# jimonld2000/AudioDenoiser

Hardware: AMD Instinct MI355X
Metric: spectrogram frames/sec (forward), 513x256 fp32 (higher is better)
Workload: dtype f32; 1 GPU; BASELINE configs[1]: batch=64 synthetic 513x256 fp32 spectrograms on one MI355X, full U-Net forward + per-clip perceptual loss; batch_per_gpu=64, global_batch=64, freq_bins=513, frames=256, parallelism=clips sharded over 1 rank(s), weights replicated, no data-path collective, lib_digest=ac1cc53c7748

## Files before the change

audiodenoiser_amd/csrc/adn_internal.h:

```cpp
#pragma once
#include <hip/hip_runtime.h>
#include <atomic>
#include <cstddef>
#include <cstdint>
#include <type_traits>

namespace adn {

template <typename T> constexpr int ACT_BLOCK = 32 / (int)sizeof(T);
template <typename T>
__host__ __device__ __forceinline__ long act_off(int C, long HW, long pix, int c)
{
    constexpr int B = ACT_BLOCK<T>;
    (void)C;
    return ((long)(c / B) * HW + pix) * B + (c % B);
}

#ifdef __HIPCC__
typedef float f32x2 __attribute__((ext_vector_type(2)));
typedef float f32x4 __attribute__((ext_vector_type(4)));
typedef float f32x16 __attribute__((ext_vector_type(16)));
typedef _Float16 f16x2 __attribute__((ext_vector_type(2)));
typedef _Float16 f16x4 __attribute__((ext_vector_type(4)));
typedef _Float16 f16x8 __attribute__((ext_vector_type(8)));
// ... 206 lines not shown
    return hipSuccess;
}
inline int device_cus()
{
    static std::atomic<int> cus{0};
    int c = cus.load(std::memory_order_relaxed);
    if (c == 0) {
        int dev = 0;
        if (hipGetDevice(&dev) != hipSuccess || hipDeviceGetAttribute(&c, hipDeviceAttributeMultiprocessorCount, dev) != hipSuccess || c < 8)
            return 0;
        c &= ~7;
        cus.store(c, std::memory_order_relaxed);
    }
    return c;
}

hipError_t launch_conv_mfma(ConvKind kind, const ConvArgs &a, bool f16, hipStream_t st);
hipError_t launch_conv_reduce(ConvKind kind, const ConvArgs &a, bool f16, hipStream_t st);
hipError_t launch_convt_reduce(const float *partial, const float *bias, float *out, int ksplit, int N, int Ho, int Wo, int Cout,
                               hipStream_t st);
constexpr int WINO_BN = 32;
hipError_t launch_wino_conv(ConvKind kind, const ConvArgs &a, hipStream_t st);
long wino_tiles(ConvArgs &a);
bool wino4_applicable(ConvKind kind, const ConvArgs &a, bool force);
long wino4_workgroups(const ConvArgs &a);
hipError_t launch_wino4_conv(ConvKind kind, const ConvArgs &a, hipStream_t st);

struct Wino3sGeom {
    int tilesY, tilesX;
    long rows;
    size_t v_bytes, m_bytes;
    long gemm_grid;
};
bool wino3s_applicable(ConvKind kind, const ConvArgs &a);
Wino3sGeom wino3s_geom(const ConvArgs &a);
hipError_t launch_wino3s_conv(ConvKind kind, const ConvArgs &a, float *V, float *M, hipStream_t st);
hipError_t launch_wino_gemm(const float *V, const void *U, float *M, long rows, int Cin, int Cout, hipStream_t st);

bool conv16_applicable(ConvKind kind, const ConvArgs &a);
hipError_t launch_conv16(ConvKind kind, const ConvArgs &a, bool resident, hipStream_t st);

bool convt16_applicable(const ConvArgs &a);
hipError_t launch_convt16(const ConvArgs &a, hipStream_t st);

hipError_t launch_conv_first(const float *x, const float *w9x64, const float *bias, void *out, bool f16,
                             int N, int H, int W, int Cin, hipStream_t st);
hipError_t launch_dot_finish(const float *planes, int nplanes, float bias, float *y, long npix, hipStream_t st);
hipError_t launch_conv_out(const void *in, bool f16, const float *w64, float bias, float *out, long npix, long HW,
                           long out_stride, hipStream_t st);
hipError_t launch_nhwc_to_nchw(const void *in, bool f16, float *out, int N, int H, int W, int C, hipStream_t st);

hipError_t launch_stft_mag(const float *audio, int n_clips, long L, int n_fft, int hop, int center, long n_frames,
                           float *out, int rows, long row_stride, long clip_stride, int quantize, hipStream_t st);
constexpr hipError_t ADN_COLD_IN_CAPTURE = hipErrorStreamCaptureUnsupported;
bool stream_is_capturing(hipStream_t st);
hipError_t stft_tables(int n_fft, const float **out, hipStream_t st);
hipError_t loss_tables(hipStream_t st);
hipError_t launch_gl_polar(const float *mag, const float *rnd, int n_clips, int F, int T, void *spec, hipStream_t st);
hipError_t launch_istft_frames(const void *spec, int n_clips, int T, int n_fft, float *buf, hipStream_t st);
hipError_t launch_istft_ola(const float *buf, int n_clips, int T, int n_fft, int hop, float *audio, hipStream_t st);
hipError_t launch_stft_complex(const float *audio, int n_clips, long L, int n_fft, int hop, int T, void *spec,
                               hipStream_t st);
struct DenoiseGeom {
    int T, K, Wd, S, V;
};
bool denoise_geom(int n_frames, int window, int overlap, DenoiseGeom *g);
hipError_t launch_denoise_windows(const void *spec, int n_clips, int F, const DenoiseGeom &g, float *out, hipStream_t st);
hipError_t launch_denoise_stitch(const float *y, int n_clips, int F, const DenoiseGeom &g, int clamp, float *out,
                                 hipStream_t st);
hipError_t launch_denoise_resynth(const float *y, const void *spec, int n_clips, long L, int n_fft, int hop,
// ... 167 lines not shown
```

audiodenoiser_amd/csrc/conv_kernels.hip:

```cpp
#include "adn_internal.h"

#include <cstdlib>

namespace adn {

namespace {

constexpr int TW = 16;
constexpr int CONVT_KG = 2, CONVT_WPE = 4;

template <typename T> struct Elem;
template <> struct Elem<float> { static constexpr int EPV = 4; };
template <> struct Elem<_Float16> { static constexpr int EPV = 8; };

template <int TH, int BN, int WM, int WN>
__device__ __forceinline__ void conv_epilogue_raw(const ConvArgs &p, f32x16 (&acc)[TH * TW / 32 / WM][BN / 32 / WN], int lane, int wave,
                                                  int ct, int n, int ty, int tx)
{
    constexpr int MB = TH * TW / 32 / WM, NB = BN / 32 / WN;
    const int wm = wave / WN, wn = wave % WN;
    const int hh = lane >> 5, l31 = lane & 31;
    float *ob = static_cast<float *>(p.out) + (size_t)n * p.H * p.W * p.Cout;
#pragma unroll
    for (int j = 0; j < NB; ++j) {
// ... 250 lines not shown
    for (int j = 0; j < NB; ++j) {
        const int col = (wn * NB + j) * 32 + l31;
        const float bv = bias_r[j];
#pragma unroll
        for (int i = 0; i < MB; ++i) {
            const int pix0 = ((HALVES == 1 ? wm * MB : 0) + i) * 32 + 4 * hh;
            float v[16];
#pragma unroll
            for (int r = 0; r < 16; ++r) {
                v[r] = acc[i][j][r] + bv;
                if (EPI != CONVT2X2 && EPI != WINO_GEMM) v[r] = relu_nan(v[r]);
            }
            if constexpr (sizeof(T) == 4) {
#pragma unroll
                for (int r = 0; r < 16; ++r) stage[(pix0 + (r & 3) + 8 * (r >> 2)) * RS + col] = v[r];
            } else {
                const bool odd = l31 & 1;
#pragma unroll
                for (int r = 0; r < 16; r += 2) {
                    const float send = odd ? v[r] : v[r + 1];
                    const float recv = __shfl_xor(send, 1, 64);
                    const float lo = odd ? recv : v[r], hi = odd ? v[r + 1] : recv;
                    const int pix = pix0 + ((r + (odd ? 1 : 0)) & 3) + 8 * (r >> 2);
                    *reinterpret_cast<f16x2 *>(stage + pix * RS + (col & ~1)) = f16x2{(_Float16)lo, (_Float16)hi};
                }
            }
        }
    }
    }
    __syncthreads();

    T *outp = static_cast<T *>(p.out);
    if constexpr (EPI == CONVT2X2) {
        static_assert(BN == 128 && NT % 64 == 0, "transposed-convolution epilogue: 128 columns per workgroup");
        constexpr int BE = ACT_BLOCK<T>, NBLK = 64 / BE;
        const int Ho = 2 * p.H, Wo = 2 * p.W;
        const int ncg = p.Cout >> 6, di = ct / ncg, cg = ct - di * ncg;
        const size_t bstr = (size_t)Ho * Wo * BE;
        T *ob = outp + (size_t)n * Ho * Wo * p.Cout + (size_t)(NBLK * cg) * bstr;
        const int gxl = lane >> 2, dj = (lane >> 1) & 1, half = lane & 1;
        const int gx = tx * TW + gxl;
        constexpr int THH = TH / HALVES;
#pragma unroll
        for (int it = 0; it < NBLK * THH / (NT / 64); ++it) {
            const int run = it * (NT / 64) + wave;
            const int b8 = run / THH, py = run - b8 * THH;
            const int gy = ty * TH + hf * THH + py;
            const piece_t val = *reinterpret_cast<const piece_t *>(stage + (py * TW + gxl) * RS + dj * 64 + b8 * BE + half * EPP);
            if (gy < p.H && gx < p.W)
                *reinterpret_cast<piece_t *>(ob + b8 * bstr + ((size_t)(2 * gy + di) * Wo + 2 * gx + dj) * BE + half * EPP) = val;
        }
        if (HALVES > 1 && hf + 1 < HALVES) __syncthreads();
    } else if constexpr (EPI == WINO_GEMM) {
        static_assert(sizeof(T) == 4 && BN % 8 == 0, "Winograd GEMM: fp32");
        constexpr int HPIX = NPIX / HALVES;
        T *ob = outp + (size_t)n * p.rows * p.Cout + (size_t)ct * (BN / 8) * p.rows * 8;
#pragma unroll
        for (int it = 0; it < HPIX * PPR / NT; ++it) {
            const int id = it * NT + tid;
            const int b8 = id / (2 * HPIX), rem = id - b8 * (2 * HPIX), pix = rem >> 1, half = rem & 1;
            const long row = (long)ty * NPIX + hf * HPIX + pix;
            if (row < p.rows)
                *reinterpret_cast<piece_t *>(ob + ((size_t)b8 * p.rows + row) * 8 + half * 4) =
                    *reinterpret_cast<const piece_t *>(stage + pix * RS + b8 * 8 + half * 4);
        }
        if (HALVES > 1 && hf + 1 < HALVES) __syncthreads();
    } else if constexpr (EPI == CONV3X3_RELU_DOT) {
        static_assert(PPR <= 64 && (PPR & (PPR - 1)) == 0 && NT % PPR == 0, "pieces of a pixel must sit in one wave");
        float wv[EPP];
#pragma unroll
        for (int e = 0; e < EPP; ++e) wv[e] = p.dotw[(tid % PPR) * EPP + e];
#pragma unroll
        for (int it = 0; it < NPIX * PPR / NT; ++it) {
            const int id = it * NT + tid;
            const int pix = id / PPR, part = id - pix * PPR;
            const int gy = ty * TH + (pix >> 4), gx = tx * TW + (pix & 15);
            const piece_t val = *reinterpret_cast<const piece_t *>(stage + pix * RS + part * EPP);
            float s = 0.f;
#pragma unroll
            for (int e = 0; e < EPP; ++e) s += wv[e] * (float)val[e];
#pragma unroll
            for (int o = PPR / 2; o > 0; o >>= 1) s += __shfl_xor(s, o, 64);
            if (part == 0 && gy < p.H && gx < p.W) p.dot_out[((size_t)n * p.H + gy) * p.W + gx] = s + p.dot_bias;
        }
// ... 481 lines not shown
#pragma unroll
        for (int a = 0; a < 2; ++a)
#pragma unroll
            for (int b = 0; b < 2; ++b) {
                const int gy = 2 * by + a, gx = 2 * bx + b;
                if (gy >= H || gx >= W) continue;
                const f32x4 v = finish(gy, gx);
                mx.x = max_nan(mx.x, v.x); mx.y = max_nan(mx.y, v.y); mx.z = max_nan(mx.z, v.z); mx.w = max_nan(mx.w, v.w);
            }
        if (by < H / 2 && bx < W / 2)
            *reinterpret_cast<Tx4 *>(pool + (size_t)n * (H / 2) * (W / 2) * Cout +
                                     act_off<T>(Cout, (long)(H / 2) * (W / 2), (long)by * (W / 2) + bx, c4)) = as_t(mx);
    }
}

template <typename T>
hipError_t launch_conv_mfma_t(ConvKind kind, const ConvArgs &a, hipStream_t st)
{
    if constexpr (sizeof(T) == 2) {
        if (a.ksplit > 1) {
            if (kind != CONV3X3_RELU) return hipErrorInvalidValue;
            return launch_dma_cfg<T, 32, 64, 8, 1, 9, 1, CONV3X3_RELU, 4, 0, 1>(a, st);
        }
        if (kind == CONVT2X2) return launch_dma_cfg<T, 8, 128, 2, 2, 1, CONVT_KG, CONVT2X2, CONVT_WPE>(a, st);
        if (kind == CONV3X3_RELU_DOT) {
            if (a.nct != 1 || !a.dotw || !a.dot_out) return hipErrorInvalidValue;
            return launch_dma_cfg<T, 32, 64, 8, 1, 9, 1, CONV3X3_RELU_DOT, 4>(a, st);
        }
        if (kind == CONV3X3_RELU_POOL) return launch_dma_cfg<T, 32, 64, 8, 1, 9, 1, CONV3X3_RELU_POOL, 4>(a, st);
        return launch_dma_cfg<T, 32, 64, 8, 1, 9, 1, CONV3X3_RELU, 4>(a, st);
    } else {
        if (kind == CONV3X3_RELU_DOT) return hipErrorInvalidValue;
        if (kind == CONVT2X2) {
            if (a.split && a.ksplit > 1) return launch_dma_cfg<T, 8, 128, 2, 2, 1, CONVT_KG, CONVT2X2, 3, 1, 1>(a, st);
            if (a.ksplit > 1) return hipErrorInvalidValue;
            if (a.split) return launch_dma_cfg<T, 8, 128, 2, 2, 1, CONVT_KG, CONVT2X2, 3, 1>(a, st);
            return launch_dma_cfg<T, 8, 128, 2, 2, 1, CONVT_KG, CONVT2X2, CONVT_WPE>(a, st);
        }
        if (a.Cout == 64) {
            if (kind == CONV3X3_RELU_POOL) return launch_cfg<T, 16, 64, 4, 1, 9, 1, CONV3X3_RELU_POOL>(a, st);
            return launch_cfg<T, 16, 64, 4, 1, 9, 1, CONV3X3_RELU>(a, st);
        }
        if (kind == CONV3X3_RELU_POOL) return launch_cfg<T, 8, 128, 2, 2, 9, 1, CONV3X3_RELU_POOL>(a, st);
        return launch_cfg<T, 8, 128, 2, 2, 9, 1, CONV3X3_RELU>(a, st);
    }
}

}

ConvGeom conv_geom(ConvKind kind, int Cout, bool f16)
{
    const int cpg = f16 ? 16 : 8;
    if (kind == CONVT2X2) return ConvGeom{8, 128, CONVT_KG * cpg};
    if (f16) return ConvGeom{32, 64, cpg};
    if (Cout == 64) return ConvGeom{16, 64, cpg};
    return ConvGeom{8, 128, cpg};
}

long conv_mfma_tiles(ConvKind kind, bool f16, ConvArgs &a)
{
    const ConvGeom g = conv_geom(kind, a.Cout, f16);
    a.tilesY = (a.H + g.TH - 1) / g.TH;
    a.tilesX = (a.W + TW - 1) / TW;
    a.nct = (kind == CONVT2X2 ? 4 * a.Cout : a.Cout) / g.BN;
    return conv_workgroups(a);
}

hipError_t launch_conv_mfma(ConvKind kind, const ConvArgs &a, bool f16, hipStream_t st)
{
    return f16 ? launch_conv_mfma_t<_Float16>(kind, a, st) : launch_conv_mfma_t<float>(kind, a, st);
}

hipError_t launch_wino_gemm(const float *V, const void *U, float *M, long rows, int Cin, int Cout, hipStream_t st)
{
    if (!V || !U || !M || rows < 1 || rows >= (1L << 25) || Cin < 16 || (Cin & 15) || Cout < 128 || (Cout & 127)) return hipErrorInvalidValue;
    ConvArgs a{};
    a.N = 36;
    a.W = TW;
    a.H = (int)((rows + TW - 1) / TW);
    a.rows = rows;
    a.s0 = ConvSrc{V, a.H, a.W, Cin, 0, 0};
    a.s1 = ConvSrc{V, 0, 0, 0, 0, 0};
    a.nchunk0 = a.nchunk = Cin / 16;
    a.wpk = U;
    a.out = M;
    a.Cout = Cout;
    a.ksplit = 1;
    a.split = 1;
    a.tilesY = (a.H + 7) / 8;
    a.tilesX = 1;
    a.nct = Cout / 128;
    return launch_dma_cfg<float, 8, 128, 2, 2, 1, CONVT_KG, WINO_GEMM, 3, 1>(a, st);
}

template <typename T>
static hipError_t launch_conv_reduce_t(bool pl, const ConvArgs &a, unsigned blocks, hipStream_t st)
{
    if (pl)
        hipLaunchKernelGGL((conv_reduce_kernel<T, true>), dim3(blocks), dim3(256), 0, st, a.partial, a.bias, static_cast<T *>(a.out),
                           static_cast<T *>(a.pool), a.ksplit, a.N, a.H, a.W, a.Cout);
    else
        hipLaunchKernelGGL((conv_reduce_kernel<T, false>), dim3(blocks), dim3(256), 0, st, a.partial, a.bias, static_cast<T *>(a.out),
                           static_cast<T *>(nullptr), a.ksplit, a.N, a.H, a.W, a.Cout);
    return hipGetLastError();
}

hipError_t launch_conv_reduce(ConvKind kind, const ConvArgs &a, bool f16, hipStream_t st)
{
    const bool pl = kind == CONV3X3_RELU_POOL;
    if (a.ksplit < 2 || a.ksplit > ADN_MAX_KSPLIT || !a.partial || (a.Cout & (f16 ? 15 : 3)) || (kind != CONV3X3_RELU && !pl) || (pl && !a.pool))
        return hipErrorInvalidValue;
    const long items = pl ? (long)a.N * ((a.H + 1) / 2) * ((a.W + 1) / 2) * (a.Cout / 4) : (long)a.N * a.H * a.W * (a.Cout / 4);
    const long blocks = (items + 255) / 256;
    if (items <= 0 || blocks > 0x7fffffffL) return hipErrorInvalidValue;
    return f16 ? launch_conv_reduce_t<_Float16>(pl, a, (unsigned)blocks, st) : launch_conv_reduce_t<float>(pl, a, (unsigned)blocks, st);
}

hipError_t launch_convt_reduce(const float *partial, const float *bias, float *out, int ksplit, int N, int Ho, int Wo, int Cout,
                               hipStream_t st)
{
    const long n4 = (long)N * Ho * Wo * Cout / 4;
    const long blocks = (n4 + 255) / 256;
    if (ksplit < 2 || ksplit > ADN_MAX_KSPLIT || (Cout & 7) || blocks <= 0 || blocks > 0x7fffffffL) return hipErrorInvalidValue;
    hipLaunchKernelGGL(convt_reduce_kernel, dim3((unsigned)blocks), dim3(256), 0, st, reinterpret_cast<const f32x4 *>(partial), bias,
// ... 69 lines not shown
```

audiodenoiser_amd/csrc/unet.hip:

```cpp
#include "adn_host.h"

#include <algorithm>
#include <cmath>
#include <cstdlib>
#include <cstring>
#include <memory>
#include <vector>

using adn::aligned_to;
using adn::DeviceGuard;
using adn::fail;
using adn::fail_hip;

namespace {

constexpr float BN_EPS = 1e-5f;
constexpr int CH[5] = {64, 128, 256, 512, 1024};

enum LayerKind { CONV3, CONVT };
struct LayerDesc {
    LayerKind kind;
    int level;
    int C0, C1;
    int Cout;
};
constexpr int N_CONV3 = 17, N_CONVT = 4, N_LAYERS = N_CONV3 + N_CONVT;
struct LayerTable {
    LayerDesc v[N_LAYERS];
    int n;
};
constexpr LayerTable make_layers()
{
    LayerTable t{};
    for (int l = 0; l <= 4; ++l) {
        if (l > 0) t.v[t.n++] = LayerDesc{CONV3, l, CH[l - 1], 0, CH[l]};
        t.v[t.n++] = LayerDesc{CONV3, l, CH[l], 0, CH[l]};
    }
    for (int l = 3; l >= 0; --l) {
        t.v[t.n++] = LayerDesc{CONVT, l + 1, CH[l + 1], 0, CH[l]};
        t.v[t.n++] = LayerDesc{CONV3, l, CH[l], CH[l], CH[l]};
        t.v[t.n++] = LayerDesc{CONV3, l, CH[l], 0, CH[l]};
    }
    return t;
}
constexpr LayerTable NET = make_layers();
static_assert(NET.n == N_LAYERS && NET.v[0].Cout == 64 && NET.v[8].C0 == 1024 && NET.v[9].kind == CONVT && NET.v[N_LAYERS - 1].Cout == 64,
              "layer table: 9 layers down to the bottleneck, then 4 x (convT, conv, conv)");
static_assert(6 * (1 + N_CONV3) + 2 * N_CONVT + 2 == ADN_N_WEIGHT_TENSORS, "layer table does not match the weight tensor list");
static_assert(1 + N_LAYERS + 1 == ADN_N_LAUNCHES, "layer table does not match the timing slots");

struct LayerWeights {
    size_t w_off, b_off;
    size_t w4_off;
    size_t w3_off;
    size_t w16_off;
    size_t braw_off;
};

}

struct adn_unet {
    int device = 0;
    float *dev = nullptr;
    size_t dev_floats = 0;
    size_t first_w = 0, first_b = 0;
    LayerWeights lw[N_LAYERS] = {};
    size_t out_w = 0;
    size_t zero_off = 0;
    float out_b = 0.f;
    std::vector<float> out_bias;
    int in_ch = 1, n_classes = 1;
    std::vector<hipEvent_t> events;
    int timing_max = 0, timing_count = 0;
    bool f16 = false;
    bool use_wino = true;
    bool use_wino4 = true, force_wino4 = false;
    bool allow_split = false;
    bool convt_split = true;
    int f16_conv = 1;
    int f16_convt = 1;
    bool f16_fuse_first = true;
    bool batch_invariant = false;
    long auto_grid = 192, auto_grid64 = 512;
    int wino_gemm = 1;
    long gemm_grid = 1536;
};

namespace {

void bn_fold(const float *b, const float *gamma, const float *beta, const float *mean, const float *var, int C,
             std::vector<float> &scale, std::vector<float> &bias)
{
    scale.resize(C);
    bias.resize(C);
    for (int c = 0; c < C; ++c) {
        const float s = gamma[c] / std::sqrt(var[c] + BN_EPS);
        scale[c] = s;
        bias[c] = (b[c] - mean[c]) * s + beta[c];
    }
}

template <typename T>
void pack_conv3x3(const float *w , const std::vector<float> &scale, int Cin, int Cout, T *dst)
{
    constexpr int EPV = 16 / sizeof(T);
    const adn::ConvGeom g = adn::conv_geom(adn::CONV3X3_RELU, Cout, sizeof(T) == 2);
    const int BN = g.BN, KC = g.KC, KG = KC / (2 * EPV);
    const int nct = Cout / BN, nchunk = Cin / KC;
    size_t o = 0;
    for (int ct = 0; ct < nct; ++ct)
        for (int ch = 0; ch < nchunk; ++ch)
            for (int tap = 0; tap < 9; ++tap)
                for (int s = 0; s < KG; ++s)
                    for (int h = 0; h < 2; ++h)
                        for (int n = 0; n < BN; ++n) {
                            const int co = ct * BN + n;
                            for (int kk = 0; kk < EPV; ++kk) {
                                const int ci = ch * KC + 2 * EPV * s + EPV * h + kk;
// ... 105 lines not shown
                            dst[(((((size_t)ct * nchunk + ch) * 16 + cb) * 4 + g) * 16 + c16) * 8 + e] =
                                (_Float16)w[(((size_t)ci * Cout + co) * 2 + di) * 2 + dj];
                        }
            }
}

inline uint16_t bf16_rne(float f)
{
    uint32_t u;
    std::memcpy(&u, &f, 4);
    if ((u & 0x7fffffffu) > 0x7f800000u) return (uint16_t)((u >> 16) | 0x40);
    u += 0x7fffu + ((u >> 16) & 1u);
    return (uint16_t)(u >> 16);
}
inline float bf16_to_float(uint16_t b)
{
    const uint32_t u = (uint32_t)b << 16;
    float f;
    std::memcpy(&f, &u, 4);
    return f;
}
inline void split3_host(float v, uint16_t (&t)[3])
{
    uint16_t hi = bf16_rne(v);
    if ((hi & 0x7fffu) == 0x7f80u && std::isfinite(v)) hi = (uint16_t)((hi & 0x8000u) | 0x7f7fu);
    const float r1 = v - bf16_to_float(hi);
    const uint16_t mid = bf16_rne(r1);
    const float r2 = r1 - bf16_to_float(mid);
    t[0] = hi;
    t[1] = mid;
    t[2] = bf16_rne(r2);
}

void pack_wino4_split(const float *w , const std::vector<float> &scale, int Cin, int Cout, uint16_t *dst)
{
    const int nct = Cout / 128, nchunk = Cin / 16;
    for (int co = 0; co < Cout; ++co)
        for (int ci = 0; ci < Cin; ++ci) {
            float U[36];
            wino4_u(w + ((size_t)co * Cin + ci) * 9, scale[co], U);
            const int ct = co / 128, n = co % 128, ch = ci / 16, hh = (ci % 16) / 8, kk = ci % 8;
            for (int pos = 0; pos < 36; ++pos) {
                uint16_t t[3];
                split3_host(U[pos], t);
                uint16_t *slab = dst + (((size_t)pos * nct + ct) * nchunk + ch) * (3 * 2 * 128 * 8);
                for (int plane = 0; plane < 3; ++plane) slab[((plane * 2 + hh) * 128 + n) * 8 + kk] = t[plane];
            }
        }
}

void pack_convt_split(const float *w , int Cin, int Cout, uint16_t *dst)
{
    const int BN = 128, KC = 16;
    const int ncol = 4 * Cout, nct = ncol / BN, nchunk = Cin / KC;
    size_t o = 0;
    for (int ct = 0; ct < nct; ++ct)
        for (int ch = 0; ch < nchunk; ++ch)
            for (int plane = 0; plane < 3; ++plane)
                for (int h = 0; h < 2; ++h)
                    for (int n = 0; n < BN; ++n) {
                        int ij, co;
                        adn::convt_column(ct * BN + n, Cout, ij, co);
                        for (int kk = 0; kk < 8; ++kk) {
                            const int ci = ch * KC + 8 * h + kk;
                            uint16_t t[3];
                            split3_host(w[((size_t)ci * Cout + co) * 4 + ij], t);
                            dst[o++] = t[plane];
                        }
                    }
}


adn::ConvArgs geom_args(const LayerDesc &d, bool f16, bool wino, int N, int H, int W)
{
    const adn::ConvKind kind = d.kind == CONVT ? adn::CONVT2X2 : adn::CONV3X3_RELU;
    adn::ConvArgs a{};
    a.s0.C = d.C0;
    a.s1.C = d.C1;
    a.N = N;
    a.H = H;
    a.W = W;
    a.Cout = d.Cout;
    a.ksplit = 1;
    const int kc = adn::conv_geom(kind, d.Cout, f16).KC;
    a.nchunk0 = d.C0 / kc;
    a.nchunk = (d.C0 + d.C1) / kc;
// ... 70 lines not shown
    }
    a.wpk = h->dev + L.w_off;
    a.wpk4 = (h->use_wino && h->use_wino4 && L.w4_off) ? h->dev + L.w4_off : (h->f16 && L.w16_off) ? h->dev + L.w16_off : nullptr;
    a.bias = h->dev + L.b_off;
    a.out = out;
    a.pool = pool;
    return a;
}

adn::ConvArgs convt_args(const adn_unet *h, const Plan &p, int i, const void *in, void *out)
{
    const LayerDesc &d = NET.v[i];
    const int H = p.H[d.level], W = p.W[d.level];
    adn::ConvArgs a = geom_args(d, h->f16, false, p.N, H, W);
    a.s0 = adn::ConvSrc{in, H, W, d.C0, 0, 0};
    a.s1 = adn::ConvSrc{in, 0, 0, 0, 0, 0};
    a.wpk = h->dev + h->lw[i].w_off;
    a.bias = h->dev + h->lw[i].b_off;
    a.out = out;
    a.split = h->convt_split ? 1 : 0;
    return a;
}


enum Conv3Kernel {
    DIRECT,
    CONV16,
    WINO2,
    WINO4,
    WINO3S
};
struct WinoScratch {
    const void *U = nullptr;
    float *V = nullptr, *M = nullptr;
    size_t v_bytes = 0, m_bytes = 0;
};
struct Conv3Choice {
    Conv3Kernel kernel;
    int ksplit;
    bool fuse_first;
    bool fuse_out;
};

Conv3Choice choose_conv3(const adn_unet *h, adn::ConvKind kind, const adn::ConvArgs &a, bool first = false, bool tail = false,
                         const WinoScratch &sc = WinoScratch())
{
    Conv3Choice c{DIRECT, 1, false, false};
    if (h->f16) {
        const bool c16 = a.wpk4 && adn::conv16_applicable(kind, a);
        c.fuse_out = tail && a.nct == 1;
        if (first && h->f16_fuse_first && c16) {
            c.kernel = CONV16;
            c.fuse_first = true;
            return c;
        }
        if (a.wpk4 && !h->batch_invariant && !c.fuse_out)
            c.ksplit = adn::conv16_ksplit(adn::conv_workgroups(a), a.nchunk, (size_t)a.N * a.H * a.W * a.Cout);
        if (c.ksplit == 1 && c16) c.kernel = CONV16;
        return c;
    }
    if (!h->use_wino) return c;
    c.kernel = WINO2;
    c.fuse_out = tail && a.nct == 2;
    auto done = [&]() {
        c.fuse_first = first && c.kernel == WINO2 && c.ksplit == 1;
        return c;
// ... 16 lines not shown
        if (fits && (h->wino_gemm == 2 || pinned || (automatic && g3.gemm_grid >= h->gemm_grid))) {
            c.kernel = WINO3S;
            return c;
        }
    }
    if (f4_ok && (!automatic || g4 >= thr)) {
        c.kernel = WINO4;
        return done();
    }
    if (automatic && can_split) c.ksplit = adn::wino_ksplit(g2, a.nchunk);
    if (automatic && can_split && f4_ok) {
        const int ks4 = adn::wino4_ksplit(g4, a.nchunk);
        if (ks4 > 1) {
            const double out_mb = (double)a.N * a.H * a.W * a.Cout * 4.0 * 1e-6;
            auto reduce_us = [&](int ks) { return ks > 1 ? 4.0 + (ks + 1) * out_mb / 8.0 : 0.0; };
            const double t4 = 12.0 + 2.79 * (a.nchunk / ks4) * (double)((g4 * ks4 + 255) / 256) + reduce_us(ks4);
            const double t2 = 8.0 + 2.06 * (a.nchunk / c.ksplit) * (double)((g2 * c.ksplit + 511) / 512) + reduce_us(c.ksplit);
            if (t4 < t2) {
                c.kernel = WINO4;
                c.ksplit = ks4;
            }
        }
    }
    return done();
}

hipError_t launch_conv3_kernels(const adn_unet *h, adn::ConvKind kind, const Conv3Choice &c, adn::ConvArgs a, float *partial, hipStream_t st,
                                const WinoScratch &sc)
{
    if (c.fuse_out) kind = adn::CONV3X3_RELU_DOT;
    switch (c.kernel) {
    case WINO3S:
        a.wpk = sc.U;
        return adn::launch_wino3s_conv(kind, a, sc.V, sc.M, st);
    case CONV16:
        a.wpk = a.wpk4;
        a.nchunk0 = a.s0.C / 32;
        a.nchunk = (a.s0.C + a.s1.C) / 32;
        if (c.fuse_first) a.nchunk0 = a.nchunk = 2;
        return adn::launch_conv16(kind, a, c.fuse_first || (a.s0.C + a.s1.C == 64 && a.Cout == 64), st);
    case DIRECT:
        if (c.ksplit > 1) {
            adn::ConvArgs sl = a;
            sl.ksplit = c.ksplit;
            sl.out = partial;
            sl.pool = nullptr;
            hipError_t e = adn::launch_conv_mfma(adn::CONV3X3_RELU, sl, true, st);
            if (e != hipSuccess) return e;
            a.ksplit = c.ksplit;
            a.partial = partial;
            return adn::launch_conv_reduce(kind, a, true, st);
        }
        return adn::launch_conv_mfma(kind, a, h->f16, st);
    case WINO4:
        a.wpk = a.wpk4;
        [[fallthrough]];
    case WINO2:
        a.ksplit = c.ksplit;
        a.partial = partial;
        return c.kernel == WINO4 ? adn::launch_wino4_conv(kind, a, st) : adn::launch_wino_conv(kind, a, st);
    }
    return hipErrorInvalidValue;
}

inline int hip_status(hipError_t e, const char *what)
{
    return e == hipSuccess ? ADN_OK : fail_hip(e, what);
// ... 19 lines not shown
struct ConvTChoice {
    bool t16;
    int ksplit;
};

ConvTChoice choose_convt(const adn_unet *h, const LayerWeights &L, const adn::ConvArgs &a)
{
    ConvTChoice c{false, 1};
    if (h->f16) {
        c.t16 = L.w16_off && adn::convt16_applicable(a);
        return c;
    }
    if (h->convt_split && !h->batch_invariant)
        c.ksplit = adn::convt_ksplit(adn::conv_workgroups(a), a.nchunk, (size_t)a.N * (2 * a.H) * (2 * a.W) * a.Cout);
    return c;
}

hipError_t launch_convt_kernels(const adn_unet *h, const LayerWeights &L, const ConvTChoice &c, adn::ConvArgs a, float *partial, hipStream_t st)
{
    if (c.t16) {
        a.wpk = h->dev + L.w16_off;
        a.bias = h->dev + L.braw_off;
        return adn::launch_convt16(a, st);
    }
    if (c.ksplit > 1) {
        float *out = static_cast<float *>(a.out);
        a.ksplit = c.ksplit;
        a.out = partial;
        a.bias = h->dev + h->zero_off;
        hipError_t e = adn::launch_conv_mfma(adn::CONVT2X2, a, h->f16, st);
        if (e != hipSuccess) return e;
        return adn::launch_convt_reduce(partial, h->dev + L.braw_off, out, c.ksplit, a.N, 2 * a.H, 2 * a.W, a.Cout, st);
    }
    return adn::launch_conv_mfma(adn::CONVT2X2, a, h->f16, st);
}

int launch_convt(const adn_unet *h, int layer, const ConvTChoice &c, const adn::ConvArgs &a, float *partial, size_t part_bytes, hipStream_t st)
{
    if (int rc = check_part(layer, c.ksplit, (size_t)a.N * (2 * a.H) * (2 * a.W) * a.Cout, part_bytes)) return rc;
    return hip_status(launch_convt_kernels(h, h->lw[layer], c, a, partial, st), "launch_convt");
}


int forward_impl(adn_unet *h, const float *x, float *y, int N, int F, int T, void *workspace, size_t ws_bytes,
                 float *const *taps, hipStream_t st)
{
    if (!h || !x || !y) return fail(ADN_ERR_INVALID, "adn_unet_forward: null handle/x/y");
    Plan p;
    if (!make_plan(N, F, T, h->f16, p)) return fail(ADN_ERR_INVALID, "adn_unet_forward: need N>=1, F,T>=16 and F*T<2^27");
    if (!workspace || ws_bytes < p.total)
        return fail(ADN_ERR_WORKSPACE, "adn_unet_forward: workspace too small (see adn_unet_workspace_bytes)");
    if (!aligned_to(workspace, 16)) return fail(ADN_ERR_INVALID, "adn_unet_forward: workspace must be 16-byte aligned");
    if (!aligned_to(x, 4) || !aligned_to(y, 4)) return fail(ADN_ERR_INVALID, "adn_unet_forward: x and y must be 4-byte aligned");
    DeviceGuard guard(h->device);
    if (guard.err != hipSuccess) return fail_hip(guard.err, "hipSetDevice");

    char *ws = static_cast<char *>(workspace);
    void *tA = ws + p.tA, *tB = ws + p.tB;
    float *part = reinterpret_cast<float *>(ws + p.part);
    const bool f16 = h->f16;
    const bool timed = h->timing_max > 0 && h->timing_count < h->timing_max && !taps;
    hipEvent_t *ev = timed ? h->events.data() + (size_t)h->timing_count * (ADN_N_LAUNCHES + 1) : nullptr;
    int evi = 0;
#define ADN_MARK()                                          \
    do {                                                    \
        if (timed) ADN_HIP(hipEventRecord(ev[evi++], st));  \
    } while (0)
#define ADN_TRY(call)                                       \
    do {                                                    \
        if (int rc_ = (call)) return rc_;                   \
    } while (0)

    auto export_tap = [&](int idx, const void *buf, int layer) -> hipError_t {
        if (!taps || !taps[idx]) return hipSuccess;
        const LayerDesc &d = NET.v[layer];
        return adn::launch_nhwc_to_nchw(buf, f16, taps[idx], N, p.H[d.level], p.W[d.level], d.Cout, st);
    };
    int i = 0;
    auto wino_scratch = [&](int li) {
        WinoScratch sc;
        const LayerDesc &d = NET.v[li];
        if (f16 || !h->lw[li].w3_off) return sc;
        const size_t full = (size_t)N * p.H[0] * p.W[0] * 64 * sizeof(float);
        const size_t front = (size_t)N * p.H[d.level] * p.W[d.level] * std::max(std::max(d.C0, d.C1), d.Cout) * sizeof(float);
        if (front >= full) return sc;
        sc.U = h->dev + h->lw[li].w3_off;
        sc.V = reinterpret_cast<float *>(static_cast<char *>(tA) + front);
        sc.M = reinterpret_cast<float *>(static_cast<char *>(tB) + front);
        sc.v_bytes = sc.m_bytes = full - front;
        return sc;
    };

    const void *cur = tA;
    for (int l = 0; l < 4; ++l) {
        void *skip = ws + p.skip[l], *pool = ws + p.pool[l];
        if (l > 0) {
            const WinoScratch sc = wino_scratch(i);
            const adn::ConvArgs a = conv_args(h, p, i++, ws + p.pool[l - 1], nullptr, 0, 0, tA, nullptr);
            ADN_MARK();
            ADN_TRY(launch_conv3(h, i - 1, adn::CONV3X3_RELU, choose_conv3(h, adn::CONV3X3_RELU, a, false, false, sc), a, part, p.part_bytes, st, sc));
        }
        const WinoScratch sc = wino_scratch(i);
        adn::ConvArgs a = conv_args(h, p, i++, cur, nullptr, 0, 0, skip, pool);
        const Conv3Choice c = choose_conv3(h, adn::CONV3X3_RELU_POOL, a, l == 0 && h->in_ch == 1, false, sc);
        if (l == 0) {
            ADN_MARK();
            if (c.fuse_first) {
                a.s0 = adn::ConvSrc{x, p.H[0], p.W[0], 1, 0, 0};
                a.firstw = h->dev + h->first_w;
                a.firstb = h->dev + h->first_b;
            } else {
                ADN_HIP(adn::launch_conv_first(x, h->dev + h->first_w, h->dev + h->first_b, tA, f16, N, p.H[0], p.W[0], h->in_ch, st));
            }
        }
        ADN_MARK();
        ADN_TRY(launch_conv3(h, i - 1, adn::CONV3X3_RELU_POOL, c, a, part, p.part_bytes, st, sc));
        ADN_HIP(export_tap(l, skip, i - 1));
    }
    {
// ... 60 lines not shown
    if (n_tensors != ADN_N_WEIGHT_TENSORS) return fail(ADN_ERR_INVALID, "adn_unet_create: expected 118 tensors");
    for (int i = 0; i < n_tensors; ++i)
        if (!t[i]) return fail(ADN_ERR_INVALID, "adn_unet_create: null tensor pointer");
    int ndev = 0;
    if (hipGetDeviceCount(&ndev) != hipSuccess || ndev <= 0) return fail(ADN_ERR_NO_DEVICE, "no HIP device visible");
    if (device < 0 || device >= ndev) return fail(ADN_ERR_INVALID, "adn_unet_create: bad device index");
    return ADN_OK;
}

int check_device_arch(int device)
{
    hipDeviceProp_t prop;
    ADN_HIP(hipGetDeviceProperties(&prop, device));
    if (std::strncmp(prop.gcnArchName, "gfx950", 6) != 0)
        return fail(ADN_ERR_NO_DEVICE, std::string("libadn is built for gfx950 only, device is ") + prop.gcnArchName);
    return ADN_OK;
}

void read_switches(adn_unet &h)
{
    if (const char *algo = std::getenv("ADN_CONV_ALGO"))
        h.use_wino = std::strcmp(algo, "direct") != 0;
    if (h.f16) h.use_wino = false;
    if (const char *sk = std::getenv("ADN_WINO_SPLITK")) h.allow_split = std::atoi(sk) != 0;
    if (const char *cs = std::getenv("ADN_CONVT_SPLIT")) h.convt_split = std::atoi(cs) != 0;
    if (const char *bi = std::getenv("ADN_BATCH_INVARIANT")) h.batch_invariant = std::atoi(bi) != 0;
    if (const char *ff = std::getenv("ADN_F16_FIRST")) h.f16_fuse_first = std::atoi(ff) != 0;
    if (const char *fc = std::getenv("ADN_F16_CONV")) h.f16_conv = std::atoi(fc) == 32 ? 0 : 1;
    if (const char *ft = std::getenv("ADN_F16_CONVT")) h.f16_convt = std::strcmp(ft, "dma") == 0 ? 0 : 1;
    if (const char *ag = std::getenv("ADN_AUTO_GRID")) h.auto_grid = std::atol(ag);
    if (const char *ag = std::getenv("ADN_AUTO_GRID64")) h.auto_grid64 = std::atol(ag);
    if (h.f16) h.convt_split = false;
    if (const char *wg = std::getenv("ADN_WINO_GEMM")) h.wino_gemm = std::atoi(wg) == 2 ? 2 : std::atoi(wg) != 0;
    if (const char *wt = std::getenv("ADN_WINO_TILE")) {
        h.use_wino4 = std::atoi(wt) != 2;
        h.force_wino4 = std::atoi(wt) == 4;
    }
}

void pack_weights(adn_unet &h, const float *const *t, std::vector<float> &host)
{
    auto reserve = [&](size_t n) {
        const size_t at = host.size();
        host.resize(at + ((n + 63) & ~size_t(63)), 0.f);
        return at;
    };
    auto halfs = [&](size_t off) { return reinterpret_cast<_Float16 *>(host.data() + off); };
    std::vector<float> scale, bias;
    bn_fold(t[1], t[2], t[3], t[4], t[5], 64, scale, bias);
    h.first_w = reserve((size_t)h.in_ch * 9 * 64);
    for (int ci = 0; ci < h.in_ch; ++ci)
        for (int tap = 0; tap < 9; ++tap)
            for (int co = 0; co < 64; ++co)
                host[h.first_w + ((size_t)ci * 9 + tap) * 64 + co] = t[0][((size_t)co * h.in_ch + ci) * 9 + tap] * scale[co];
    h.first_b = reserve(64);
    std::memcpy(host.data() + h.first_b, bias.data(), sizeof(float) * 64);
    int ti = 6;
    for (int i = 0; i < N_LAYERS; ++i) {
        const LayerDesc &d = NET.v[i];
        LayerWeights &L = h.lw[i];
        const int Cin = d.C0 + d.C1, Cout = d.Cout;
        const size_t n16 = ((size_t)(d.kind == CONVT ? 4 : 9) * Cin * Cout + 1) / 2;
        if (d.kind == CONVT) {
            if (h.f16) {
                L.w_off = reserve(n16);
                pack_convt<_Float16>(t[ti], Cin, Cout, halfs(L.w_off));
                if (h.f16_convt != 0 && Cin % 128 == 0 && Cout % 64 == 0) {
                    L.w16_off = reserve(n16);
                    pack_convt16(t[ti], Cin, Cout, halfs(L.w16_off));
                    L.braw_off = reserve(Cout);
                    std::memcpy(host.data() + L.braw_off, t[ti + 1], sizeof(float) * Cout);
                }
            } else if (h.convt_split) {
                L.w_off = reserve(3 * n16);
                pack_convt_split(t[ti], Cin, Cout, reinterpret_cast<uint16_t *>(host.data() + L.w_off));
                L.braw_off = reserve(Cout);
                std::memcpy(host.data() + L.braw_off, t[ti + 1], sizeof(float) * Cout);
            } else {
                L.w_off = reserve((size_t)4 * Cin * Cout);
                pack_convt<float>(t[ti], Cin, Cout, host.data() + L.w_off);
            }
            L.b_off = reserve((size_t)4 * Cout);
            for (int col = 0; col < 4 * Cout; ++col) {
                int ij, c;
                adn::convt_column(col, Cout, ij, c);
                host[L.b_off + col] = t[ti + 1][c];
            }
            ti += 2;
            continue;
        }
        bn_fold(t[ti + 1], t[ti + 2], t[ti + 3], t[ti + 4], t[ti + 5], Cout, scale, bias);
        if (h.f16 && h.f16_conv != 0 && Cin % 32 == 0 && Cout % 64 == 0) {
            L.w16_off = reserve(n16);
            pack_conv16(t[ti], scale, Cin, Cout, halfs(L.w16_off));
        }
        if (h.use_wino) {
            L.w_off = reserve((size_t)16 * Cin * Cout);
            pack_wino3x3(t[ti], scale, Cin, Cout, adn::WINO_BN, host.data() + L.w_off);
            if (h.use_wino4) {
                L.w4_off = reserve((size_t)36 * Cin * Cout);
                pack_wino4_3x3(t[ti], scale, Cin, Cout, host.data() + L.w4_off);
                if (h.wino_gemm && d.level >= 3 && Cin >= 512 && Cin % 16 == 0 && Cout % 128 == 0) {
                    L.w3_off = reserve((size_t)36 * Cin * Cout * 3 / 2);
                    pack_wino4_split(t[ti], scale, Cin, Cout, reinterpret_cast<uint16_t *>(host.data() + L.w3_off));
                }
            }
        } else if (h.f16) {
            L.w_off = reserve(n16);
            pack_conv3x3<_Float16>(t[ti], scale, Cin, Cout, halfs(L.w_off));
        } else {
            L.w_off = reserve((size_t)9 * Cin * Cout);
            pack_conv3x3<float>(t[ti], scale, Cin, Cout, host.data() + L.w_off);
        }
        L.b_off = reserve(Cout);
        std::memcpy(host.data() + L.b_off, bias.data(), sizeof(float) * Cout);
        ti += 6;
    }
    h.zero_off = reserve(4 * 512);
    h.out_w = reserve((size_t)64 * h.n_classes);
    std::memcpy(host.data() + h.out_w, t[ti], sizeof(float) * 64 * h.n_classes);
    h.out_bias.assign(t[ti + 1], t[ti + 1] + h.n_classes);
    h.out_b = t[ti + 1][0];
}

struct UnetDeleter {
    void operator()(adn_unet *h) const
    {
        {
            DeviceGuard guard(h->device);
            for (hipEvent_t e : h->events) (void)hipEventDestroy(e);
            if (h->dev) (void)hipFree(h->dev);
        }
        delete h;
    }
};

}
// ... 9 lines not shown
{
    return adn_unet_create_general(handle, device, t, n_tensors, dtype, 1, 1);
}

int adn_unet_channels(const adn_unet *h, int *in_channels, int *num_classes)
{
    if (!h || !in_channels || !num_classes) return fail(ADN_ERR_INVALID, "adn_unet_channels: null argument");
    *in_channels = h->in_ch;
    *num_classes = h->n_classes;
    return ADN_OK;
}

int adn_unet_set_batch_invariant(adn_unet *h, int on)
{
    if (!h) return fail(ADN_ERR_INVALID, "adn_unet_set_batch_invariant: null handle");
    h->batch_invariant = on != 0;
    return ADN_OK;
}

int adn_unet_create_general(adn_unet **handle, int device, const float *const *t, int n_tensors, int dtype, int in_channels,
                            int num_classes)
{
    if (int rc = check_create_args(handle, device, t, n_tensors, dtype, in_channels, num_classes)) return rc;
    DeviceGuard guard(device);
    if (guard.err != hipSuccess) return fail_hip(guard.err, "hipSetDevice");
    if (int rc = check_device_arch(device)) return rc;

    std::unique_ptr<adn_unet, UnetDeleter> h(new adn_unet());
    h->device = device;
    h->in_ch = in_channels;
    h->n_classes = num_classes;
    h->f16 = dtype == ADN_DTYPE_F16;
    read_switches(*h);
    std::vector<float> host;
    pack_weights(*h, t, host);
    h->dev_floats = host.size();
    hipError_t e = hipMalloc(&h->dev, host.size() * sizeof(float));
    if (e != hipSuccess) return fail_hip(e, "hipMalloc(weights)");
    e = hipMemcpy(h->dev, host.data(), host.size() * sizeof(float), hipMemcpyHostToDevice);
    if (e != hipSuccess) return fail_hip(e, "hipMemcpy(weights)");
    *handle = h.release();
    return ADN_OK;
}

int adn_unet_set_timing(adn_unet *h, int max_forwards)
{
    if (!h || max_forwards < 0 || max_forwards > 4096) return fail(ADN_ERR_INVALID, "adn_unet_set_timing: bad argument");
    DeviceGuard guard(h->device);
    if (guard.err != hipSuccess) return fail_hip(guard.err, "hipSetDevice");
    for (hipEvent_t e : h->events) (void)hipEventDestroy(e);
    h->events.clear();
    h->timing_max = 0;
    h->timing_count = 0;
    h->events.resize((size_t)max_forwards * (ADN_N_LAUNCHES + 1));
    for (size_t i = 0; i < h->events.size(); ++i) ADN_HIP(hipEventCreate(&h->events[i]));
    h->timing_max = max_forwards;
    return ADN_OK;
}

int adn_unet_get_timing(adn_unet *h, int index, float *ms)
{
    if (!h || !ms || index < 0 || index >= h->timing_count) return fail(ADN_ERR_INVALID, "adn_unet_get_timing: no such forward");
    DeviceGuard guard(h->device);
    if (guard.err != hipSuccess) return fail_hip(guard.err, "hipSetDevice");
    hipEvent_t *ev = h->events.data() + (size_t)index * (ADN_N_LAUNCHES + 1);
    ADN_HIP(hipEventSynchronize(ev[ADN_N_LAUNCHES]));
// ... 33 lines not shown
```

audiodenoiser_amd/csrc/wino3s_kernels.hip:

```cpp
#include "adn_internal.h"

namespace adn {

namespace {

constexpr int NT = 256;

__global__ __launch_bounds__(NT) void wino3s_input_kernel(const ConvArgs p, float *__restrict__ V, int tilesY, int tilesX, long rows)
{
    const long id = (long)blockIdx.x * NT + threadIdx.x;
    const long row = id >> 1;
    const int half = (int)(id & 1), cb = blockIdx.y;
    if (row >= rows) return;
    const int tx = (int)(row % tilesX);
    const long r2 = row / tilesX;
    const int ty = (int)(r2 % tilesY), n = (int)(r2 / tilesY);
    const bool second = cb >= p.s0.C / 8;
    const ConvSrc &s = second ? p.s1 : p.s0;
    const int cbl = second ? cb - p.s0.C / 8 : cb;
    const float *src = static_cast<const float *>(s.ptr) + ((size_t)n * (s.C / 8) + cbl) * ((size_t)s.H * s.W * 8) + half * 4;
    const int y0 = 4 * ty - 1 - s.offY, x0 = 4 * tx - 1 - s.offX;
    f32x4 d[6][6];
#pragma unroll
    for (int a = 0; a < 6; ++a)
// ... 62 lines not shown
#pragma unroll
            for (int b = 0; b < 2; ++b) {
                const int py = 2 * ty + a, px = 2 * tx + b;
                const f32x4 mx = __builtin_elementwise_maximum(__builtin_elementwise_maximum(y[2 * a][2 * b], y[2 * a][2 * b + 1]),
                                                               __builtin_elementwise_maximum(y[2 * a + 1][2 * b], y[2 * a + 1][2 * b + 1]));
                if (py < Hp && px < Wp) *reinterpret_cast<f32x4 *>(pb + ((size_t)py * Wp + px) * 8) = mx;
            }
    }
}

}

bool wino3s_applicable(ConvKind kind, const ConvArgs &a)
{
    if (kind != CONV3X3_RELU && kind != CONV3X3_RELU_POOL) return false;
    if (kind == CONV3X3_RELU_POOL && !a.pool) return false;
    const int Cin = a.s0.C + a.s1.C;
    if (a.firstw || a.ksplit > 1 || Cin < 16 || (Cin & 15) || (a.s0.C & 7) || a.Cout < 128 || (a.Cout & 127)) return false;
    return a.N >= 1 && a.H >= 1 && a.W >= 1 && wino3s_geom(a).rows < (1L << 25);
}

Wino3sGeom wino3s_geom(const ConvArgs &a)
{
    Wino3sGeom g{};
    g.tilesY = (a.H + 3) / 4;
    g.tilesX = (a.W + 3) / 4;
    g.rows = (long)a.N * g.tilesY * g.tilesX;
    g.v_bytes = (size_t)36 * g.rows * (a.s0.C + a.s1.C) * sizeof(float);
    g.m_bytes = (size_t)36 * g.rows * a.Cout * sizeof(float);
    g.gemm_grid = 36 * ((g.rows + 127) / 128) * (a.Cout / 128);
    return g;
}

hipError_t launch_wino3s_conv(ConvKind kind, const ConvArgs &a, float *V, float *M, hipStream_t st)
{
    if (!wino3s_applicable(kind, a) || !V || !M || !a.wpk || !a.bias || !a.out) return hipErrorInvalidValue;
    const Wino3sGeom g = wino3s_geom(a);
    const long bx = (2 * g.rows + NT - 1) / NT;
    const int Cin = a.s0.C + a.s1.C;
    hipLaunchKernelGGL(wino3s_input_kernel, dim3((unsigned)bx, (unsigned)(Cin / 8)), dim3(NT), 0, st, a, V, g.tilesY, g.tilesX, g.rows);
    hipError_t e = hipGetLastError();
    if (e != hipSuccess) return e;
    e = launch_wino_gemm(V, a.wpk, M, g.rows, Cin, a.Cout, st);
    if (e != hipSuccess) return e;
    if (kind == CONV3X3_RELU_POOL)
        hipLaunchKernelGGL(wino3s_output_kernel<true>, dim3((unsigned)bx, (unsigned)(a.Cout / 8)), dim3(NT), 0, st, a, M, g.tilesY,
                           g.tilesX, g.rows);
    else
        hipLaunchKernelGGL(wino3s_output_kernel<false>, dim3((unsigned)bx, (unsigned)(a.Cout / 8)), dim3(NT), 0, st, a, M, g.tilesY,
                           g.tilesX, g.rows);
    return hipGetLastError();
}

}
```

Measured before the change: 519,600 frames/s.

## Add 256-column tiles for split-precision Winograd GEMM and transposed convolution

Adds 256-column workgroup tile variants, with 4 or 8 waves, for the split-bf16 Winograd GEMM and the transposed-convolution MFMA kernels. Weights are repacked per tile width, and a second packed copy is kept for transposed convs. The wider tile is picked by default when the channel count divides evenly, and for transposed convs only when the grid is large. The goal is to reuse each loaded activation tile across more output columns and cut the number of workgroups, at the cost of more registers and LDS per workgroup, lower occupancy, and extra weight memory.

```diff
diff --git a/audiodenoiser_amd/csrc/adn_internal.h b/audiodenoiser_amd/csrc/adn_internal.h
--- a/audiodenoiser_amd/csrc/adn_internal.h
+++ b/audiodenoiser_amd/csrc/adn_internal.h
@@ -262,10 +262,12 @@
     size_t v_bytes, m_bytes;
     long gemm_grid;
 };
+enum SplitTile { SPLIT_BN128 = 0, SPLIT_BN256 = 1, SPLIT_BN256W8 = 2 };
+inline int split_tile_bn(SplitTile t) { return t == SPLIT_BN128 ? 128 : 256; }
 bool wino3s_applicable(ConvKind kind, const ConvArgs &a);
 Wino3sGeom wino3s_geom(const ConvArgs &a);
-hipError_t launch_wino3s_conv(ConvKind kind, const ConvArgs &a, float *V, float *M, hipStream_t st);
-hipError_t launch_wino_gemm(const float *V, const void *U, float *M, long rows, int Cin, int Cout, hipStream_t st);
+hipError_t launch_wino3s_conv(ConvKind kind, const ConvArgs &a, float *V, float *M, SplitTile tile, hipStream_t st);
+hipError_t launch_wino_gemm(const float *V, const void *U, float *M, long rows, int Cin, int Cout, SplitTile tile, hipStream_t st);
 
 bool conv16_applicable(ConvKind kind, const ConvArgs &a);
 hipError_t launch_conv16(ConvKind kind, const ConvArgs &a, bool resident, hipStream_t st);
diff --git a/audiodenoiser_amd/csrc/conv_kernels.hip b/audiodenoiser_amd/csrc/conv_kernels.hip
--- a/audiodenoiser_amd/csrc/conv_kernels.hip
+++ b/audiodenoiser_amd/csrc/conv_kernels.hip
@@ -306,24 +306,35 @@
 
     T *outp = static_cast<T *>(p.out);
     if constexpr (EPI == CONVT2X2) {
-        static_assert(BN == 128 && NT % 64 == 0, "transposed-convolution epilogue: 128 columns per workgroup");
+        static_assert((BN == 128 || BN == 256) && NT % 64 == 0, "transposed-convolution epilogue: 128 or 256 columns per workgroup");
         constexpr int BE = ACT_BLOCK<T>, NBLK = 64 / BE;
+        constexpr int NSUB = BN / 128;
         const int Ho = 2 * p.H, Wo = 2 * p.W;
-        const int ncg = p.Cout >> 6, di = ct / ncg, cg = ct - di * ncg;
+        const int ncg = p.Cout >> 6;
+        int di[NSUB], cg[NSUB];
+#pragma unroll
+        for (int sub = 0; sub < NSUB; ++sub) {
+            di[sub] = (ct * NSUB + sub) / ncg;
+            cg[sub] = (ct * NSUB + sub) - di[sub] * ncg;
+        }
         const size_t bstr = (size_t)Ho * Wo * BE;
-        T *ob = outp + (size_t)n * Ho * Wo * p.Cout + (size_t)(NBLK * cg) * bstr;
+        T *ob[NSUB];
+#pragma unroll
+        for (int sub = 0; sub < NSUB; ++sub) ob[sub] = outp + (size_t)n * Ho * Wo * p.Cout + (size_t)(NBLK * cg[sub]) * bstr;
         const int gxl = lane >> 2, dj = (lane >> 1) & 1, half = lane & 1;
         const int gx = tx * TW + gxl;
         constexpr int THH = TH / HALVES;
 #pragma unroll
-        for (int it = 0; it < NBLK * THH / (NT / 64); ++it) {
-            const int run = it * (NT / 64) + wave;
-            const int b8 = run / THH, py = run - b8 * THH;
-            const int gy = ty * TH + hf * THH + py;
-            const piece_t val = *reinterpret_cast<const piece_t *>(stage + (py * TW + gxl) * RS + dj * 64 + b8 * BE + half * EPP);
-            if (gy < p.H && gx < p.W)
-                *reinterpret_cast<piece_t *>(ob + b8 * bstr + ((size_t)(2 * gy + di) * Wo + 2 * gx + dj) * BE + half * EPP) = val;
-        }
+        for (int sub = 0; sub < NSUB; ++sub)
+#pragma unroll
+            for (int it = 0; it < NBLK * THH / (NT / 64); ++it) {
+                const int run = it * (NT / 64) + wave;
+                const int b8 = run / THH, py = run - b8 * THH;
+                const int gy = ty * TH + hf * THH + py;
+                const piece_t val = *reinterpret_cast<const piece_t *>(stage + (py * TW + gxl) * RS + dj * 64 + b8 * BE + half * EPP + sub * 128);
+                if (gy < p.H && gx < p.W)
+                    *reinterpret_cast<piece_t *>(ob[sub] + b8 * bstr + ((size_t)(2 * gy + di[sub]) * Wo + 2 * gx + dj) * BE + half * EPP) = val;
+            }
         if (HALVES > 1 && hf + 1 < HALVES) __syncthreads();
     } else if constexpr (EPI == WINO_GEMM) {
         static_assert(sizeof(T) == 4 && BN % 8 == 0, "Winograd GEMM: fp32");
@@ -871,8 +882,11 @@
     } else {
         if (kind == CONV3X3_RELU_DOT) return hipErrorInvalidValue;
         if (kind == CONVT2X2) {
+            if (a.split > 1 && a.ksplit > 1) return hipErrorInvalidValue;
             if (a.split && a.ksplit > 1) return launch_dma_cfg<T, 8, 128, 2, 2, 1, CONVT_KG, CONVT2X2, 3, 1, 1>(a, st);
             if (a.ksplit > 1) return hipErrorInvalidValue;
+            if (a.split == 1 + SPLIT_BN256) return launch_dma_cfg<T, 8, 256, 2, 2, 1, CONVT_KG, CONVT2X2, 2, 1>(a, st);
+            if (a.split == 1 + SPLIT_BN256W8) return launch_dma_cfg<T, 8, 256, 2, 4, 1, CONVT_KG, CONVT2X2, 2, 1>(a, st);
             if (a.split) return launch_dma_cfg<T, 8, 128, 2, 2, 1, CONVT_KG, CONVT2X2, 3, 1>(a, st);
             return launch_dma_cfg<T, 8, 128, 2, 2, 1, CONVT_KG, CONVT2X2, CONVT_WPE>(a, st);
         }
@@ -910,9 +924,10 @@
     return f16 ? launch_conv_mfma_t<_Float16>(kind, a, st) : launch_conv_mfma_t<float>(kind, a, st);
 }
 
-hipError_t launch_wino_gemm(const float *V, const void *U, float *M, long rows, int Cin, int Cout, hipStream_t st)
-{
-    if (!V || !U || !M || rows < 1 || rows >= (1L << 25) || Cin < 16 || (Cin & 15) || Cout < 128 || (Cout & 127)) return hipErrorInvalidValue;
+hipError_t launch_wino_gemm(const float *V, const void *U, float *M, long rows, int Cin, int Cout, SplitTile tile, hipStream_t st)
+{
+    const int BN = split_tile_bn(tile);
+    if (!V || !U || !M || rows < 1 || rows >= (1L << 25) || Cin < 16 || (Cin & 15) || Cout < BN || Cout % BN) return hipErrorInvalidValue;
     ConvArgs a{};
     a.N = 36;
     a.W = TW;
@@ -928,7 +943,9 @@
     a.split = 1;
     a.tilesY = (a.H + 7) / 8;
     a.tilesX = 1;
-    a.nct = Cout / 128;
+    a.nct = Cout / BN;
+    if (tile == SPLIT_BN256) return launch_dma_cfg<float, 8, 256, 2, 2, 1, CONVT_KG, WINO_GEMM, 2, 1>(a, st);
+    if (tile == SPLIT_BN256W8) return launch_dma_cfg<float, 8, 256, 2, 4, 1, CONVT_KG, WINO_GEMM, 2, 1>(a, st);
     return launch_dma_cfg<float, 8, 128, 2, 2, 1, CONVT_KG, WINO_GEMM, 3, 1>(a, st);
 }
 
diff --git a/audiodenoiser_amd/csrc/unet.hip b/audiodenoiser_amd/csrc/unet.hip
--- a/audiodenoiser_amd/csrc/unet.hip
+++ b/audiodenoiser_amd/csrc/unet.hip
@@ -53,8 +53,10 @@
     size_t w_off, b_off;
     size_t w4_off;
     size_t w3_off;
+    adn::SplitTile w3_tile;
     size_t w16_off;
     size_t braw_off;
+    size_t wt_off;
 };
 
 }
@@ -84,6 +86,8 @@
     long auto_grid = 192, auto_grid64 = 512;
     int wino_gemm = 1;
     long gemm_grid = 1536;
+    int split_bn = -1;
+    long convt_wide_grid = 2048;
 };
 
 namespace {
@@ -255,26 +259,26 @@
     t[2] = bf16_rne(r2);
 }
 
-void pack_wino4_split(const float *w , const std::vector<float> &scale, int Cin, int Cout, uint16_t *dst)
-{
-    const int nct = Cout / 128, nchunk = Cin / 16;
+void pack_wino4_split(const float *w , const std::vector<float> &scale, int Cin, int Cout, int BN, uint16_t *dst)
+{
+    const int nct = Cout / BN, nchunk = Cin / 16;
     for (int co = 0; co < Cout; ++co)
         for (int ci = 0; ci < Cin; ++ci) {
             float U[36];
             wino4_u(w + ((size_t)co * Cin + ci) * 9, scale[co], U);
-            const int ct = co / 128, n = co % 128, ch = ci / 16, hh = (ci % 16) / 8, kk = ci % 8;
+            const int ct = co / BN, n = co % BN, ch = ci / 16, hh = (ci % 16) / 8, kk = ci % 8;
             for (int pos = 0; pos < 36; ++pos) {
                 uint16_t t[3];
                 split3_host(U[pos], t);
-                uint16_t *slab = dst + (((size_t)pos * nct + ct) * nchunk + ch) * (3 * 2 * 128 * 8);
-                for (int plane = 0; plane < 3; ++plane) slab[((plane * 2 + hh) * 128 + n) * 8 + kk] = t[plane];
+                uint16_t *slab = dst + (((size_t)pos * nct + ct) * nchunk + ch) * ((size_t)3 * 2 * BN * 8);
+                for (int plane = 0; plane < 3; ++plane) slab[((plane * 2 + hh) * BN + n) * 8 + kk] = t[plane];
             }
         }
 }
 
-void pack_convt_split(const float *w , int Cin, int Cout, uint16_t *dst)
-{
-    const int BN = 128, KC = 16;
+void pack_convt_split(const float *w , int Cin, int Cout, int BN , uint16_t *dst)
+{
+    const int KC = 16;
     const int ncol = 4 * Cout, nct = ncol / BN, nchunk = Cin / KC;
     size_t o = 0;
     for (int ct = 0; ct < nct; ++ct)
@@ -411,6 +415,7 @@
 };
 struct WinoScratch {
     const void *U = nullptr;
+    adn::SplitTile tile = adn::SPLIT_BN128;
     float *V = nullptr, *M = nullptr;
     size_t v_bytes = 0, m_bytes = 0;
 };
@@ -493,7 +498,7 @@
     switch (c.kernel) {
     case WINO3S:
         a.wpk = sc.U;
-        return adn::launch_wino3s_conv(kind, a, sc.V, sc.M, st);
+        return adn::launch_wino3s_conv(kind, a, sc.V, sc.M, sc.tile, st);
     case CONV16:
         a.wpk = a.wpk4;
         a.nchunk0 = a.s0.C / 32;
@@ -579,6 +584,11 @@
         if (e != hipSuccess) return e;
         return adn::launch_convt_reduce(partial, h->dev + L.braw_off, out, c.ksplit, a.N, 2 * a.H, 2 * a.W, a.Cout, st);
     }
+    if (a.split && L.wt_off && (h->split_bn >= 0 || adn::conv_workgroups(a) >= h->convt_wide_grid)) {
+        a.split = 1 + L.w3_tile;
+        a.wpk = h->dev + L.wt_off;
+        a.nct /= 2;
+    }
     return adn::launch_conv_mfma(adn::CONVT2X2, a, h->f16, st);
 }
 
@@ -632,6 +642,7 @@
         const size_t front = (size_t)N * p.H[d.level] * p.W[d.level] * std::max(std::max(d.C0, d.C1), d.Cout) * sizeof(float);
         if (front >= full) return sc;
         sc.U = h->dev + h->lw[li].w3_off;
+        sc.tile = h->lw[li].w3_tile;
         sc.V = reinterpret_cast<float *>(static_cast<char *>(tA) + front);
         sc.M = reinterpret_cast<float *>(static_cast<char *>(tB) + front);
         sc.v_bytes = sc.m_bytes = full - front;
@@ -758,10 +769,19 @@
     if (const char *ag = std::getenv("ADN_AUTO_GRID64")) h.auto_grid64 = std::atol(ag);
     if (h.f16) h.convt_split = false;
     if (const char *wg = std::getenv("ADN_WINO_GEMM")) h.wino_gemm = std::atoi(wg) == 2 ? 2 : std::atoi(wg) != 0;
+    if (const char *sb = std::getenv("ADN_SPLIT_BN"))
+        h.split_bn = !std::strcmp(sb, "128") ? adn::SPLIT_BN128 : !std::strcmp(sb, "256") ? adn::SPLIT_BN256 : !std::strcmp(sb, "256w8") ? adn::SPLIT_BN256W8 : -2;
     if (const char *wt = std::getenv("ADN_WINO_TILE")) {
         h.use_wino4 = std::atoi(wt) != 2;
         h.force_wino4 = std::atoi(wt) == 4;
     }
+}
+
+adn::SplitTile split_tile(const adn_unet &h, const LayerDesc &d)
+{
+    if ((d.kind == CONVT ? 4 * d.Cout : d.Cout) % 256) return adn::SPLIT_BN128;
+    if (h.split_bn >= 0) return static_cast<adn::SplitTile>(h.split_bn);
+    return d.kind == CONVT && d.Cout < 128 ? adn::SPLIT_BN128 : adn::SPLIT_BN256;
 }
 
 void pack_weights(adn_unet &h, const float *const *t, std::vector<float> &host)
@@ -799,7 +819,12 @@
                 }
             } else if (h.convt_split) {
                 L.w_off = reserve(3 * n16);
-                pack_convt_split(t[ti], Cin, Cout, reinterpret_cast<uint16_t *>(host.data() + L.w_off));
+                pack_convt_split(t[ti], Cin, Cout, 128, reinterpret_cast<uint16_t *>(host.data() + L.w_off));
+                L.w3_tile = split_tile(h, d);
+                if (L.w3_tile != adn::SPLIT_BN128) {
+                    L.wt_off = reserve(3 * n16);
+                    pack_convt_split(t[ti], Cin, Cout, adn::split_tile_bn(L.w3_tile), reinterpret_cast<uint16_t *>(host.data() + L.wt_off));
+                }
                 L.braw_off = reserve(Cout);
                 std::memcpy(host.data() + L.braw_off, t[ti + 1], sizeof(float) * Cout);
             } else {
@@ -828,7 +853,8 @@
                 pack_wino4_3x3(t[ti], scale, Cin, Cout, host.data() + L.w4_off);
                 if (h.wino_gemm && d.level >= 3 && Cin >= 512 && Cin % 16 == 0 && Cout % 128 == 0) {
                     L.w3_off = reserve((size_t)36 * Cin * Cout * 3 / 2);
-                    pack_wino4_split(t[ti], scale, Cin, Cout, reinterpret_cast<uint16_t *>(host.data() + L.w3_off));
+                    L.w3_tile = split_tile(h, d);
+                    pack_wino4_split(t[ti], scale, Cin, Cout, adn::split_tile_bn(L.w3_tile), reinterpret_cast<uint16_t *>(host.data() + L.w3_off));
                 }
             }
         } else if (h.f16) {
@@ -904,6 +930,7 @@
     h->n_classes = num_classes;
     h->f16 = dtype == ADN_DTYPE_F16;
     read_switches(*h);
+    if (h->split_bn < -1) return fail(ADN_ERR_INVALID, "adn_unet_create: ADN_SPLIT_BN must be 128, 256 or 256w8");
     std::vector<float> host;
     pack_weights(*h, t, host);
     h->dev_floats = host.size();
diff --git a/audiodenoiser_amd/csrc/wino3s_kernels.hip b/audiodenoiser_amd/csrc/wino3s_kernels.hip
--- a/audiodenoiser_amd/csrc/wino3s_kernels.hip
+++ b/audiodenoiser_amd/csrc/wino3s_kernels.hip
@@ -118,7 +118,7 @@
     return g;
 }
 
-hipError_t launch_wino3s_conv(ConvKind kind, const ConvArgs &a, float *V, float *M, hipStream_t st)
+hipError_t launch_wino3s_conv(ConvKind kind, const ConvArgs &a, float *V, float *M, SplitTile tile, hipStream_t st)
 {
     if (!wino3s_applicable(kind, a) || !V || !M || !a.wpk || !a.bias || !a.out) return hipErrorInvalidValue;
     const Wino3sGeom g = wino3s_geom(a);
@@ -127,7 +127,7 @@
     hipLaunchKernelGGL(wino3s_input_kernel, dim3((unsigned)bx, (unsigned)(Cin / 8)), dim3(NT), 0, st, a, V, g.tilesY, g.tilesX, g.rows);
     hipError_t e = hipGetLastError();
     if (e != hipSuccess) return e;
-    e = launch_wino_gemm(V, a.wpk, M, g.rows, Cin, a.Cout, st);
+    e = launch_wino_gemm(V, a.wpk, M, g.rows, Cin, a.Cout, tile, st);
     if (e != hipSuccess) return e;
     if (kind == CONV3X3_RELU_POOL)
         hipLaunchKernelGGL(wino3s_output_kernel<true>, dim3((unsigned)bx, (unsigned)(a.Cout / 8)), dim3(NT), 0, st, a, M, g.tilesY,
```

Result: faster. 532,700 frames/s, median of 6 (+2.5%).
